# taintpro98/rnd-semantic-segmentation

Hardware: AMD Instinct MI355X
Metric: train images/sec at 769x769 bf16 (DeepLabV2-ResNet101 + ASPP) (higher is better)
Workload: dtype bf16; 1 GPU; train_src.py DeepLabV2-R101 bf16, 769x769 synthetic Cityscapes crops, batch 8 per GPU, 1xMI355X; global_batch=8, parallelism=dp1, weights=formula (synthetic), hip_graph_replay=False

## Files before the change

### rnd_semantic_segmentation_amd/csrc/elementwise.hip

```cpp
#include "mi_common.h"
#include <mutex>
#include <stdlib.h>
#include <string.h>

static thread_local char g_err[512] = "";

int mi_set_error(int code, const char* fmt, ...) {
    va_list ap;
    va_start(ap, fmt);
    vsnprintf(g_err, sizeof(g_err), fmt, ap);
    va_end(ap);
    return code;
}

const MiSwitches& mi_sw() {
    static MiSwitches sw;
    static std::once_flag once;
    std::call_once(once, [] {
        auto env = [](const char* name, int dflt) {
            const char* e = getenv(name);
            return e ? atoi(e) : dflt;
        };
        sw.igemm_staged = env("MI_IGEMM_STAGED", 1);
        sw.igemm_pp = env("MI_IGEMM_PP", 1);
        sw.igemm_pp_mink = env("MI_IGEMM_PP_MINK", 512);
        sw.igemm_mt = env("MI_IGEMM_MT", 0);
        sw.igemm_bn = env("MI_IGEMM_BN", 0);
        sw.igemm_pref = env("MI_IGEMM_PREF", 1);
        sw.pp_korder = env("MI_IGEMM_PP_KORDER", 1);
#ifdef MI_EXPERIMENTS
        sw.pp_loop = env("MI_IGEMM_PP_LOOP", 0);
#else
        sw.pp_loop = 0;
#endif
        sw.igemm_pw = env("MI_IGEMM_PW", 0);
        sw.wgrad_q3_slots = env("MI_WGRAD_Q3_SLOTS", 512);
        sw.wgrad_q3_slots_beside = env("MI_WGRAD_Q3_SLOTS_BESIDE", 448);
        sw.wgrad_s4_slots = env("MI_WGRAD_S4_SLOTS", 512);
        if (sw.wgrad_s4_slots < 64) sw.wgrad_s4_slots = 512;
        sw.wgrad_ti256 = env("MI_WGRAD_TI256", -1);
        sw.wgrad_p3 = env("MI_WGRAD_P3", 0);
        sw.wgrad_q3 = env("MI_WGRAD_Q3", 1);
        sw.wgrad_s4 = env("MI_WGRAD_S4", 1);
        sw.gconv_bn128 = env("MI_GCONV_BN128", 0);
        sw.gconv_kc = env("MI_GCONV_KC", 0);
        sw.gconv_remap = env("MI_GCONV_REMAP", 1);
        sw.gconv_ks2_wgs = env("MI_GCONV_KS2_WGS", 320);
        sw.gconv_kc32_wgs = env("MI_GCONV_KC32_WGS", 1536);
        sw.gconv_bn32_wgs = env("MI_GCONV_BN32_WGS", 256);
        sw.gconv_bn_any = env("MI_GCONV_BN_ANY", 1);
        sw.gconv_bn_c = env("MI_GCONV_BN_C", 64);
        sw.gconv_bn_force = env("MI_GCONV_BN_FORCE", 0);
        sw.gconv3_wgs = env("MI_GCONV3_WGS", 512);
#ifdef MI_EXPERIMENTS
        sw.gconv_dbg = env("MI_GC_DBG", 0);
        sw.gw_dbg = env("MI_GW_DBG", 0);
#else
        sw.gconv_dbg = sw.gw_dbg = 0;
#endif
        sw.gwm_steps = env("MI_GWM_STEPS", 48);
        if (sw.gwm_steps < 1) sw.gwm_steps = 48;
        sw.gwm_fused3 = env("MI_GWM_FUSED3", 1);
        sw.gwgrad3 = env("MI_GWGRAD3", 1);
#ifdef MI_EXPERIMENTS
        sw.p3_dbg = env("MI_P3_DBG", 0);
#else
        sw.p3_dbg = 0;
#endif
        sw.pp_trace_wg = env("MI_PP_TRACE_WG", 0);
        sw.stem_direct = env("MI_STEM_DIRECT", 1);
        sw.stem_pool_wgrad = env("MI_STEM_POOL_WGRAD", 1);
        sw.head_mask = env("MI_HEAD_MASK", 1);
        sw.sgd_pack = env("MI_SGD_PACK", 1);
        sw.stem_wgrad_splits = env("MI_STEM_WGRAD_SPLITS", 512);
        if (sw.stem_wgrad_splits < 1 || sw.stem_wgrad_splits > 4096) sw.stem_wgrad_splits = 512;
    });
// ... 337 lines not shown
```

### rnd_semantic_segmentation_amd/csrc/igemm_tn.hip

```cpp
#include "wgrad_common.h"
#include <stdlib.h>

namespace {

constexpr int TO = 128, TI = 128, KP = 64;
constexpr int ROWB = 256;
constexpr int TILE_BYTES = KP * ROWB;
constexpr int STAGE_BYTES = 2 * TILE_BYTES;
constexpr int LDS_BYTES = 2 * STAGE_BYTES;

__device__ __attribute__((aligned(256))) uint32_t g_zero_page_tn[64];

struct WgradParams {
    const __bf16* dY;
    const __bf16* X;
    float* slab;
    int M, O, I, T;
    int Ho, Wo, Ha, Wa;
    int ksz, stride, pad, dil;
    int S, rows_per_split;
    int o_tiles, i_tiles;
};

template <int OFF>
// ... 140 lines not shown
    const int wi = wave & 1, wo_ = wave >> 1;
    f32x4 acc[4][4];
#pragma unroll
    for (int a = 0; a < 4; ++a)
#pragma unroll
        for (int b = 0; b < 4; ++b) acc[a][b] = f32x4{0.f, 0.f, 0.f, 0.f};

    const int g = lane >> 4, q = (lane & 15) >> 2, pc = lane & 3;
    const int rsw = (((g & 1) * 4 + q) << 1);
    const int row_off = (g * 4 + q) * ROWB + (pc & 1) * 8;
    const unsigned lds0 = lds_address(smem);
    auto compute = [&](int buf) {
        const unsigned sy = lds0 + buf * STAGE_BYTES + row_off;
        const unsigned sx = sy + TILE_BYTES;
#pragma unroll
        for (int ks = 0; ks < 2; ++ks) tn_frag_mfma(sy + (ks * 32) * ROWB, sx + (ks * 32) * ROWB, wi, wo_, pc, rsw, acc);
    };

    if (nk > 0) {
        stage(0);
        asm volatile("s_waitcnt vmcnt(0)" ::: "memory");
        __syncthreads();
        for (int kt = 0; kt < nk; ++kt) {
            const int cur = kt & 1;
            if (kt + 1 < nk) stage(cur ^ 1);
            compute(cur);
            asm volatile("s_waitcnt vmcnt(0)" ::: "memory");
            __syncthreads();
        }
    }
    slab_store(p.slab + ((long)(split * p.T + t) * p.O) * p.I, p.I, p.O, p.I, o0 + wo_ * 64, i0 + wi * 64, lane, acc);
}

constexpr int KP4 = 32, SLOT4 = 2 * KP4 * ROWB, NSLOT4 = 4, LDS4_BYTES = NSLOT4 * SLOT4;

__global__ __launch_bounds__(256, 2) void wgrad_s4_kernel(WgradParams p) {
    extern __shared__ __attribute__((aligned(16))) char smem[];
    const int tid = threadIdx.x, lane = tid & 63;
    const int wave = __builtin_amdgcn_readfirstlane(tid >> 6);
    const WgDecode wg = wg_decode<TO, TI, KP4>(blockIdx.x, p.o_tiles * p.i_tiles * p.S, p.o_tiles, p.i_tiles, 1, p.M, p.rows_per_split);
    const int split = wg.split, o0 = wg.o0, i0 = wg.i0, m_begin = wg.m_begin, m_end = wg.m_end, nk = wg.nk;

    const int prow = lane >> 4, pch = lane & 15;
    const long rows = m_end > m_begin ? m_end - m_begin : 0;
    const __amdgpu_buffer_rsrc_t rs_y = __builtin_amdgcn_make_buffer_rsrc(const_cast<__bf16*>(p.dY + (long)m_begin * p.O), 0, (int)(rows * p.O * 2), 0x00020000);
    const __amdgpu_buffer_rsrc_t rs_x = __builtin_amdgcn_make_buffer_rsrc(const_cast<__bf16*>(p.X + (long)m_begin * p.I), 0, (int)(rows * p.I * 2), 0x00020000);
    unsigned vy[2], vx[2];
#pragma unroll
    for (int j = 0; j < 2; ++j) {
        const int row = (wave * 2 + j) * 4 + prow;
        const int lch = pch ^ ((row & 7) << 1);
        const int oc = o0 + lch * 8, ic = i0 + lch * 8;
        vy[j] = (unsigned)(((long)row * p.O + oc) * 2) | (oc < p.O ? 0u : 0x80000000u);
        vx[j] = (unsigned)(((long)row * p.I + ic) * 2) | (ic < p.I ? 0u : 0x80000000u);
    }
    const unsigned y_step = (unsigned)KP4 * p.O * 2, x_step = (unsigned)KP4 * p.I * 2;
    auto stage = [&](int slot) {
        char* sy = smem + slot * SLOT4 + wave * 2048;
        char* sx = sy + KP4 * ROWB;
#pragma unroll
        for (int j = 0; j < 2; ++j) {
            blds16_tn(rs_y, vy[j], sy + j * 1024);
            blds16_tn(rs_x, vx[j], sx + j * 1024);
            vy[j] += y_step;
            vx[j] += x_step;
        }
    };

    const int wi = wave & 1, wo_ = wave >> 1;
    f32x4 acc[4][4];
#pragma unroll
    for (int a = 0; a < 4; ++a)
#pragma unroll
        for (int b = 0; b < 4; ++b) acc[a][b] = f32x4{0.f, 0.f, 0.f, 0.f};
    const int g = lane >> 4, q = (lane & 15) >> 2, pc = lane & 3;
    const int rsw = (((g & 1) * 4 + q) << 1);
    const int row_off = (g * 4 + q) * ROWB + (pc & 1) * 8;
    const unsigned lds0 = lds_address(smem);
    auto compute = [&](int slot) {
        const unsigned sy = lds0 + slot * SLOT4 + row_off;
        tn_frag_mfma(sy, sy + KP4 * ROWB, wi, wo_, pc, rsw, acc);
    };

    stage(0);
    stage(1);
    stage(2);
    for (int s = 0; s < nk; ++s) {
        asm volatile("s_waitcnt vmcnt(8)" ::: "memory");
        __builtin_amdgcn_s_barrier();
        stage((s + 3) & (NSLOT4 - 1));
        compute(s & (NSLOT4 - 1));
    }
    slab_store(p.slab + ((long)split * p.O) * p.I, p.I, p.O, p.I, o0 + wo_ * 64, i0 + wi * 64, lane, acc);
}

constexpr int TI2 = 256, KP2 = 32;
constexpr int XROWB = 512;
constexpr int Y2_BYTES = KP2 * ROWB, X2_BYTES = KP2 * XROWB;
constexpr int STAGE2_BYTES = Y2_BYTES + X2_BYTES, NSTAGE2 = 3, LDS2_BYTES = NSTAGE2 * STAGE2_BYTES;

template <int MODE>
__global__ __launch_bounds__(256, 2) void wgrad_tn256_kernel(WgradParams p) {
    extern __shared__ __attribute__((aligned(16))) char smem[];
    const int tid = threadIdx.x, lane = tid & 63;
    const int wave = __builtin_amdgcn_readfirstlane(tid >> 6);
    const WgDecode wg = wg_decode<TO, TI2, KP2>(blockIdx.x, p.o_tiles * p.i_tiles * p.T * p.S, p.o_tiles, p.i_tiles, p.T, p.M, p.rows_per_split);
    const int t = wg.mid, split = wg.split, o0 = wg.o0, i0 = wg.i0, m_begin = wg.m_begin, m_end = wg.m_end, nk = wg.nk;
    const int ky = t / p.ksz, kx = t - ky * p.ksz;
    const char* zero = reinterpret_cast<const char*>(g_zero_page_tn);

    const int yrow_l = lane >> 4, ych = lane & 15, xrow_l = lane >> 5, xch = lane & 31;
    const int dys = ky * p.dil - p.pad, dxs = kx * p.dil - p.pad;
    int y_m[2], x_m[4], x_ho[4], x_wo[4];
    const char* y_ptr[2];
    const char* x_ptr[4];
    bool y_col[2], x_col[4];
    const int HoWo = p.Ho * p.Wo;
#pragma unroll
    for (int j = 0; j < 2; ++j) {
        const int row = (wave * 2 + j) * 4 + yrow_l;
        const int lch = ych ^ ((row & 7) << 1);
        y_m[j] = m_begin + row;
        y_col[j] = o0 + lch * 8 < p.O;
        y_ptr[j] = reinterpret_cast<const char*>(p.dY + (long)y_m[j] * p.O + o0 + lch * 8);
// ... 173 lines not shown
    wgrad_reduce_body(q.slab, q.dw, q.scale, q.S, q.T, q.O, q.I, q.accumulate, q.out_map, q.ncls, bx, o, tile);
}

constexpr int P3_KS = 64, P3_XROWS = 80;
constexpr int P3_DY_BYTES = P3_KS * ROWB, P3_X_BYTES = P3_XROWS * ROWB, P3_SLAB = P3_DY_BYTES + P3_X_BYTES;
constexpr int P3_LDS = 4 * P3_SLAB;
constexpr int P3_NPY = 4, P3_NPX = 5;

struct WgradP3Params {
    const __bf16* dY;
    const __bf16* X;
    float* slab;
    int O, I, H, W, d, WP, BH;
    long Q;
    int S, slabs_per_split;
    int o_tiles, i_tiles;
    int dbg;
};

#ifdef MI_EXPERIMENTS
#include "../../tools/experiments/wgrad_p3.inc"
#endif

constexpr int Q3_TO = 64;
constexpr int Q3_YROWB = 128;
constexpr int Q3_DY_BYTES = P3_KS * Q3_YROWB, Q3_STAGE = Q3_DY_BYTES + P3_X_BYTES;
constexpr int Q3_LDS = 2 * Q3_STAGE;

#ifdef MI_EXPERIMENTS
#define Q3_DBG(b) (p.dbg & (b))
#else
#define Q3_DBG(b) 0
#endif
__global__ __launch_bounds__(256, 2) void wgrad_q3_kernel(WgradP3Params p) {
    extern __shared__ __attribute__((aligned(16))) char smem[];
    const int tid = threadIdx.x, lane = tid & 63;
    const int wq = __builtin_amdgcn_readfirstlane(tid >> 6);
    const WgDecode wg = wg_decode_tile<Q3_TO, TI>(blockIdx.x, p.o_tiles * p.i_tiles * 3 * p.S, p.o_tiles, p.i_tiles, 3);
    const int ky = wg.mid, split = wg.split, o0 = wg.o0, i0 = wg.i0;
    const long q_begin = (long)split * p.slabs_per_split * P3_KS;
    long left = (p.Q - q_begin + P3_KS - 1) / P3_KS;
    const int ns = (int)(left < 0 ? 0 : (left < p.slabs_per_split ? left : p.slabs_per_split));
    const int Qi = (int)p.Q;
    const int n0 = P3_KS / p.WP, r0 = P3_KS - n0 * p.WP;
    const int pix_step = n0 * p.W + r0;

    const int yprow = lane >> 3, ypch = lane & 7;
    const char* yzero = reinterpret_cast<const char*>(g_zero_page_tn) + ypch * 16;
    const int yspan0 = wq * 16;
    const int ylch = ypch ^ ((((yspan0 + yprow) >> 1) & 3) << 1);
    const bool yok = o0 + ylch * 8 < p.O;
    const unsigned yrow_bytes = (unsigned)p.O * 2u;
    const unsigned yoff = yprow * yrow_bytes + (o0 + ylch * 8) * 2;
    const char* dy_b = reinterpret_cast<const char*>(p.dY);
    int y_q = (int)(q_begin + yspan0), y_wp, y_pix;
    {
        const int bh = y_q / p.WP;
        y_wp = y_q - bh * p.WP;
        y_pix = bh * p.W + y_wp - p.d;
    }
    const int xprow = lane >> 4, xpch = lane & 15;
    const char* xzero = reinterpret_cast<const char*>(g_zero_page_tn) + xpch * 16;
    const int dh = (ky - 1) * p.d;
    const int xspan0 = wq * 20;
    const int xlch_e = xpch ^ (((xspan0 + xprow) & 7) << 1), xlch_o = xpch ^ (((xspan0 + xprow + 4) & 7) << 1);
    const bool xok_e = i0 + xlch_e * 8 < p.I, xok_o = i0 + xlch_o * 8 < p.I;
    const unsigned xrow_bytes = (unsigned)p.I * 2u;
    const unsigned xoff_e = xprow * xrow_bytes + (i0 + xlch_e * 8) * 2, xoff_o = xprow * xrow_bytes + (i0 + xlch_o * 8) * 2;
    const char* x_b = reinterpret_cast<const char*>(p.X);
    int x_q = (int)(q_begin + xspan0 - p.d), x_wp, x_h, x_pix;
    {
        const long qs = (long)x_q + p.WP;
        const int bh = (int)(qs / p.WP) - 1;
        x_wp = (int)(qs % p.WP);
// ... 126 lines not shown
            } else {
#pragma unroll
                for (int b = 0; b < 4; ++b) asm volatile("" ::"v"(yf[b].v));
#pragma unroll
                for (int kx = 0; kx < 3; ++kx)
#pragma unroll
                    for (int a = 0; a < 2; ++a) asm volatile("" ::"v"(xf[kx][a].v));
            }
        }
    };

    if (ns > 0) {
        stage(0);
        asm volatile("s_waitcnt vmcnt(0)" ::: "memory");
        __syncthreads();
        for (int s = 0; s < ns; ++s) {
            const int cur = s & 1;
            if (s + 1 < ns && !Q3_DBG(1)) stage(cur ^ 1);
            compute(cur);
            asm volatile("s_waitcnt vmcnt(0)" ::: "memory");
            __syncthreads();
        }
    }

    if (Q3_DBG(8)) {
#pragma unroll
        for (int kx = 0; kx < 3; ++kx)
#pragma unroll
            for (int a = 0; a < 2; ++a)
#pragma unroll
                for (int b = 0; b < 4; ++b) asm volatile("" ::"v"(acc[kx][a][b]));
        return;
    }
#pragma unroll
    for (int kx = 0; kx < 3; ++kx) slab_store(p.slab + ((long)(split * 9 + ky * 3 + kx) * p.O) * p.I, p.I, p.O, p.I, o0, i0 + wq * 32, lane, acc[kx]);
}

struct P3Plan { int S, slabs_per_split; long Q; int WP, o_tiles, i_tiles; };
bool p3_plan(int B, int H, int W, int O, int I, int dil, bool force, P3Plan& pl, bool q3 = false, bool beside = false) {
    if (dil < 1 || dil > 8) return false;
    pl.WP = W + 2 * dil;
    pl.Q = (long)B * H * pl.WP;
    pl.o_tiles = q3 ? (O + Q3_TO - 1) / Q3_TO : (O + TO - 1) / TO;
    pl.i_tiles = (I + TI - 1) / TI;
    const long ns = (pl.Q + P3_KS - 1) / P3_KS;
    const int groups = pl.o_tiles * pl.i_tiles * 3;
    long S = (q3 ? (beside ? mi_sw().wgrad_q3_slots_beside : mi_sw().wgrad_q3_slots) : 256) / groups;
    if (S < 1) S = 1;
    if (S > ns) S = ns;
    pl.slabs_per_split = (int)((ns + S - 1) / S);
    pl.S = (int)((ns + pl.slabs_per_split - 1) / pl.slabs_per_split);
    if (P3_KS / pl.WP + 1 > H || pl.WP < 20 || pl.Q >= (1L << 31) - 4096) return false;
    if (force) return true;
    if (q3) return (long)O * I >= 256L * 256 && pl.slabs_per_split >= 8;
    return O >= 96 && I >= 96 && pl.slabs_per_split >= 8;
}

int pick_splits(long M, int tiles) { return wgrad_pick_splits(M, tiles, KP, 8, 6, 512, 64); }

}

extern "C" size_t mi_conv_wgrad_workspace(int B, int Ho, int Wo, int O, int I, int ksize) {
    const long M = (long)B * Ho * Wo;
    const int T = ksize * ksize;
    const int tiles = ((O + TO - 1) / TO) * ((I + TI - 1) / TI) * T;
    const int S = pick_splits(M, tiles);
    size_t need = (size_t)S * T * O * I * sizeof(float);
    if (I >= 256) {
        const int S2 = pick_splits256(M, ((O + TO - 1) / TO) * ((I + TI2 - 1) / TI2) * T);
        const size_t n2 = (size_t)S2 * T * O * I * sizeof(float);
        if (n2 > need) need = n2;
    }
    if (ksize == 1) {
        const size_t n4 = (size_t)(pick_splits256(M, tiles) > pick_splits_s4(M, tiles) ? pick_splits256(M, tiles) : pick_splits_s4(M, tiles)) * O * I * sizeof(float);
        if (n4 > need) need = n4;
    }
    if (ksize == 3) {
        P3Plan pl;
        for (int d = 1; d <= 8; d *= 2)
            for (int q3 = 0; q3 < 2; ++q3)
                if (p3_plan(B, Ho, Wo, O, I, d, true, pl, q3 != 0)) {
                    const size_t n3 = (size_t)pl.S * 9 * O * I * sizeof(float);
                    if (n3 > need) need = n3;
                }
    }
    return need;
}

template <auto KERN, int LDS, class P>
static void launch_lds(unsigned grid, unsigned block, hipStream_t st, const P& p) {
    static std::atomic<uint64_t> attr{0};
    mi_allow_dynamic_lds((const void*)KERN, LDS, attr);
    hipLaunchKernelGGL(KERN, dim3(grid), dim3(block), LDS, st, p);
}

static int launch_p3(const void* dy, const void* x, float* ws, int H, int W, int O, int I, int dil, const P3Plan& pl, int BH, hipStream_t st, bool q3 = false) {
    WgradP3Params q;
    q.dY = (const __bf16*)dy;
    q.X = (const __bf16*)x;
    q.slab = ws;
    q.O = O;
    q.I = I;
    q.H = H;
    q.W = W;
    q.d = dil;
    q.WP = pl.WP;
    q.BH = BH;
    q.Q = pl.Q;
    q.S = pl.S;
    q.slabs_per_split = pl.slabs_per_split;
    q.o_tiles = pl.o_tiles;
    q.i_tiles = pl.i_tiles;
    q.dbg = mi_sw().p3_dbg;
    const unsigned nb = (unsigned)(pl.o_tiles * pl.i_tiles * 3 * pl.S);
    if (q3) {
        launch_lds<wgrad_q3_kernel, Q3_LDS>(nb, 256, st, q);
        return 0;
    }
#ifdef MI_EXPERIMENTS
    launch_lds<wgrad_p3_kernel, P3_LDS>(nb, 512, st, q);
    return 0;
#else
    return -1;
#endif
}

struct WgradPlan {
    int kernel;
    int mode;
    int S;
    int steps;
    int step_rows;
    int o_tiles, i_tiles;
    int deferred;
    P3Plan p3;
};
static void wgrad_plan(int B, int Ha, int Wa, int I, int Ho, int Wo, int O, int ksize, int stride, int pad, int dil, int out_map, bool deferred,
                       size_t workspace_bytes, WgradPlan& w) {
    w = WgradPlan{};
    w.deferred = deferred;
    const long M = (long)B * Ho * Wo;
    const int T = ksize * ksize;
    const bool same = stride == 1 && Ha == Ho && Wa == Wo;
#ifdef MI_EXPERIMENTS
    const int p3_mode = mi_sw().wgrad_p3;
#else
    const int p3_mode = 0;
#endif
    const int q3_mode = mi_sw().wgrad_q3;
    const bool fused_ok = out_map == 0 && ksize == 3 && same && pad == dil;
    for (int q3 = 1; q3 >= 0; --q3) {
        const int mode = q3 ? (p3_mode ? 0 : q3_mode) : p3_mode;
        if (!fused_ok || !mode) continue;
        P3Plan pl;
        if (p3_plan(B, Ho, Wo, O, I, dil, mode == 2, pl, q3 != 0, q3 && deferred) && (size_t)pl.S * 9 * O * I * sizeof(float) <= workspace_bytes) {
            w.kernel = q3 ? MI_WPLAN_Q3 : MI_WPLAN_P3;
            w.S = pl.S;
            w.steps = pl.slabs_per_split;
            w.step_rows = P3_KS;
            w.o_tiles = pl.o_tiles;
            w.i_tiles = pl.i_tiles;
            w.p3 = pl;
            return;
        }
    }
    w.o_tiles = (O + TO - 1) / TO;
    const bool small32 = (long)M * (O > I ? O : I) * 2 < (1L << 31);
    const bool pointwise = same && ksize == 1 && pad == 0;
    if (use_tn256(O, I, ksize, pad, stride, Ha, Ho, Wa, Wo)) {
        w.kernel = MI_WPLAN_TN256;
        w.mode = pointwise ? 2 : 1;
        w.i_tiles = (I + TI2 - 1) / TI2;
        w.S = pick_splits256(M, w.o_tiles * w.i_tiles * T);
        w.step_rows = KP2;
    } else if (mi_sw().wgrad_s4 && pointwise && small32) {
        w.kernel = MI_WPLAN_S4;
        w.i_tiles = (I + TI - 1) / TI;
        w.S = pick_splits_s4(M, w.o_tiles * w.i_tiles);
        w.step_rows = KP4;
    } else {
        w.kernel = MI_WPLAN_TN;
        w.mode = pointwise && small32 ? 2 : (same ? 1 : 0);
        w.i_tiles = (I + TI - 1) / TI;
        w.S = pick_splits(M, w.o_tiles * w.i_tiles * T);
        w.step_rows = KP;
    }
    const long steps = (M + w.step_rows - 1) / w.step_rows;
    w.steps = (int)((steps + w.S - 1) / w.S);
}

extern "C" int mi_conv_wgrad_route(int B, int Ha, int Wa, int I, int Ho, int Wo, int O, int ksize, int stride, int pad, int dil, int out_map) {
    WgradPlan w;
    wgrad_plan(B, Ha, Wa, I, Ho, Wo, O, ksize, stride, pad, dil, out_map, false, mi_conv_wgrad_workspace(B, Ho, Wo, O, I, ksize), w);
    return w.kernel;
}

extern "C" int mi_conv_wgrad_plan(int B, int Ha, int Wa, int I, int Ho, int Wo, int O, int ksize, int stride, int pad, int dil, int out_map, int deferred,
                                  int* plan) {
    MI_REQUIRE(plan, "mi_conv_wgrad_plan: null plan");
    MI_REQUIRE(B > 0 && Ha > 0 && Wa > 0 && Ho > 0 && Wo > 0 && O > 0 && I > 0, "mi_conv_wgrad_plan: non-positive dimension");
    MI_REQUIRE(ksize == 1 || ksize == 3, "mi_conv_wgrad_plan: ksize");
    MI_REQUIRE(stride >= 1 && dil >= 1 && pad >= 0, "mi_conv_wgrad_plan: bad stride/dil/pad");
    WgradPlan w;
    wgrad_plan(B, Ha, Wa, I, Ho, Wo, O, ksize, stride, pad, dil, out_map, deferred != 0, mi_conv_wgrad_workspace(B, Ho, Wo, O, I, ksize), w);
    const int v[MI_WPLAN_LEN] = {w.kernel, w.mode, w.S, w.steps, w.step_rows, w.o_tiles, w.i_tiles, w.deferred};
    for (int k = 0; k < MI_WPLAN_LEN; ++k) plan[k] = v[k];
    return MI_OK;
}

static int wgrad_finish(WgradReduceJob* defer, hipStream_t stream, const float* slab, float* dw, const float* scale, int S, int T, int O, int I, int accumulate,
                        int out_map, int ncls, int o_real) {
    const int gx = (I + (T == 1 ? 255 : 63)) / (T == 1 ? 256 : 64);
    if (defer) {
        *defer = WgradReduceJob{slab, dw, scale, S, T, O, I, accumulate, out_map, ncls, gx, o_real};
        return MI_OK;
    }
    hipLaunchKernelGGL(wgrad_reduce_kernel, dim3((unsigned)gx, (unsigned)o_real), dim3(256), 0, stream, slab, dw, scale, S, T, O, I, accumulate, out_map, ncls);
    MI_CHECK_LAUNCH("mi_conv_wgrad reduce");
    return MI_OK;
}

static int mi_conv_wgrad_impl(const void* dy, const void* x, float* dw, int B, int Ha, int Wa, int I, int Ho, int Wo, int O,
                              int ksize, int stride, int pad, int dil, const float* scale_o, int accumulate, int out_map, int ncls,
                              size_t dw_elems, void* workspace, size_t workspace_bytes, void* stream, WgradReduceJob* defer) {
    MI_REQUIRE(dy && x && dw && workspace, "mi_conv_wgrad: null operand");
    MI_REQUIRE(B > 0 && Ha > 0 && Wa > 0 && Ho > 0 && Wo > 0, "mi_conv_wgrad: non-positive dimension");
    MI_REQUIRE(O % 8 == 0 && I % 8 == 0, "mi_conv_wgrad: O=%d, I=%d must be multiples of 8", O, I);
    MI_REQUIRE(ksize == 1 || ksize == 3, "mi_conv_wgrad: ksize");
    MI_REQUIRE(out_map == 0 || (out_map == 1 && ksize == 1), "mi_conv_wgrad: out_map 1 needs ksize 1");
    if (out_map == 1) {
        MI_REQUIRE(ncls > 0 && 36 * ncls <= MI_ASPP_KPAD && O >= 36 * ncls, "mi_conv_wgrad: out_map 1 needs 0 < 36*ncls=%d <= min(O=%d, %d)", 36 * ncls, O, MI_ASPP_KPAD);
        MI_REQUIRE(dw_elems >= (size_t)36 * ncls * I, "mi_conv_wgrad: dw holds %zu floats, the ASPP gradient needs %zu", dw_elems, (size_t)36 * ncls * I);
    } else {
        MI_REQUIRE(dw_elems >= (size_t)O * I * ksize * ksize, "mi_conv_wgrad: dw holds %zu floats, the gradient needs %zu", dw_elems, (size_t)O * I * ksize * ksize);
    }
    MI_REQUIRE(mi_aligned16(dy) && mi_aligned16(x) && mi_aligned16(workspace), "mi_conv_wgrad: alignment");
    const long M = (long)B * Ho * Wo;
    MI_REQUIRE(M < (1L << 31) && (long)B * Ha * Wa < (1L << 31), "mi_conv_wgrad: pixel count overflows int32");
    const size_t need = mi_conv_wgrad_workspace(B, Ho, Wo, O, I, ksize);
    if (workspace_bytes < need) return mi_set_error(MI_ENOMEM, "mi_conv_wgrad: workspace %zu < %zu", workspace_bytes, need);
    WgradPlan w;
    wgrad_plan(B, Ha, Wa, I, Ho, Wo, O, ksize, stride, pad, dil, out_map, defer != nullptr, workspace_bytes, w);
    if (w.kernel == MI_WPLAN_Q3 || w.kernel == MI_WPLAN_P3) {
        if (launch_p3(dy, x, (float*)workspace, Ho, Wo, O, I, dil, w.p3, B * Ho, (hipStream_t)stream, w.kernel == MI_WPLAN_Q3) != 0)
            return mi_set_error(MI_EINVAL, "mi_conv_wgrad: the 8-wave fused-row kernel exists in experiment builds only");
        MI_CHECK_LAUNCH("mi_conv_wgrad (fused 3x3 rows)");
        return wgrad_finish(defer, (hipStream_t)stream, (const float*)workspace, dw, scale_o, w.S, 9, O, I, accumulate, 0, 1, O);
    }
    WgradParams p;
    p.dY = (const __bf16*)dy;
    p.X = (const __bf16*)x;
    p.slab = (float*)workspace;
    p.M = (int)M;
    p.O = O;
    p.I = I;
    p.T = ksize * ksize;
    p.Ho = Ho;
    p.Wo = Wo;
    p.Ha = Ha;
    p.Wa = Wa;
    p.ksz = ksize;
    p.stride = stride;
    p.pad = pad;
    p.dil = dil;
    p.o_tiles = w.o_tiles;
    p.i_tiles = w.i_tiles;
    p.S = w.S;
    p.rows_per_split = w.steps * w.step_rows;
    const hipStream_t sq = (hipStream_t)stream;
    const unsigned nb = (unsigned)(p.o_tiles * p.i_tiles * p.T * p.S);
    if (w.kernel == MI_WPLAN_TN256) {
        if (w.mode == 2) launch_lds<wgrad_tn256_kernel<2>, LDS2_BYTES>(nb, 256, sq, p);
        else launch_lds<wgrad_tn256_kernel<1>, LDS2_BYTES>(nb, 256, sq, p);
        MI_CHECK_LAUNCH("mi_conv_wgrad (128 x 256 tile)");
    } else if (w.kernel == MI_WPLAN_S4) {
        launch_lds<wgrad_s4_kernel, LDS4_BYTES>(nb, 256, sq, p);
        MI_CHECK_LAUNCH("mi_conv_wgrad (1x1 deep stream)");
    } else {
        if (w.mode == 2) launch_lds<wgrad_tn_kernel<2>, LDS_BYTES>(nb, 256, sq, p);
        else if (w.mode == 1) launch_lds<wgrad_tn_kernel<1>, LDS_BYTES>(nb, 256, sq, p);
        else launch_lds<wgrad_tn_kernel<0>, LDS_BYTES>(nb, 256, sq, p);
        MI_CHECK_LAUNCH("mi_conv_wgrad");
    }
    int o_real = O;
    if (out_map == 1) o_real = 36 * ncls;
    else ncls = 1;
    return wgrad_finish(defer, (hipStream_t)stream, p.slab, dw, scale_o, p.S, p.T, O, I, accumulate, out_map, ncls, o_real);
}

extern "C" int mi_conv_wgrad(const void* dy, const void* x, float* dw, int B, int Ha, int Wa, int I, int Ho, int Wo, int O,
                             int ksize, int stride, int pad, int dil, const float* scale_o, int accumulate, int out_map, int ncls,
                             size_t dw_elems, void* workspace, size_t workspace_bytes, void* stream) {
    return mi_conv_wgrad_impl(dy, x, dw, B, Ha, Wa, I, Ho, Wo, O, ksize, stride, pad, dil, scale_o, accumulate, out_map, ncls, dw_elems, workspace, workspace_bytes,
                              stream, nullptr);
}

extern "C" size_t mi_conv_wgrad_job_bytes(void) { return sizeof(WgradReduceJob); }
extern "C" int mi_conv_wgrad_partial(const void* dy, const void* x, float* dw, int B, int Ha, int Wa, int I, int Ho, int Wo, int O,
                                     int ksize, int stride, int pad, int dil, const float* scale_o, int accumulate, int out_map, int ncls,
                                     size_t dw_elems, void* workspace, size_t workspace_bytes, void* job, void* stream) {
    MI_REQUIRE(job, "mi_conv_wgrad_partial: null job");
    return mi_conv_wgrad_impl(dy, x, dw, B, Ha, Wa, I, Ho, Wo, O, ksize, stride, pad, dil, scale_o, accumulate, out_map, ncls, dw_elems, workspace, workspace_bytes,
                              stream, (WgradReduceJob*)job);
}
extern "C" int mi_conv_wgrad_reduce(const void* jobs, int n, void* stream) {
    MI_REQUIRE(jobs && n >= 1 && n <= MI_REDUCE_MAX_JOBS, "mi_conv_wgrad_reduce: 1 .. %d jobs", MI_REDUCE_MAX_JOBS);
    WgradReduceTable tab;
    tab.n = n;
    int total = 0;
// ... 13 lines not shown
```

### rnd_semantic_segmentation_amd/csrc/mi_common.h

```cpp
#pragma once
#include <hip/hip_runtime.h>
#include <stdint.h>
#include <stdio.h>
#include <stdarg.h>
#include <atomic>
#include "../../include/mi355seg.h"

typedef __attribute__((ext_vector_type(8))) __bf16 bf16x8;
typedef __attribute__((ext_vector_type(4))) __bf16 bf16x4;
typedef __attribute__((ext_vector_type(2))) __bf16 bf16x2;
typedef __attribute__((ext_vector_type(4))) float f32x4;
typedef __attribute__((ext_vector_type(4))) short s16x4;
typedef __attribute__((ext_vector_type(4))) uint32_t u32x4;
typedef __attribute__((ext_vector_type(2))) uint32_t u32x2;

int mi_set_error(int code, const char* fmt, ...);

struct MiSwitches {
    int igemm_staged;
    int igemm_pp;
    int igemm_pp_mink;
    int igemm_mt;
    int igemm_bn;
    int igemm_pref;
    int pp_korder;
    int pp_loop;
    int igemm_pw;
    int wgrad_q3_slots;
    int wgrad_q3_slots_beside;
    int wgrad_s4_slots;
    int wgrad_ti256;
    int wgrad_p3;
    int wgrad_q3;
    int wgrad_s4;
    int gconv_bn128;
    int gconv_kc;
    int gconv_remap;
    int gconv_ks2_wgs;
    int gconv_kc32_wgs;
    int gconv_bn32_wgs;
    int gconv_bn_any;
    int gconv_bn_c;
    int gconv_bn_force;
    int gconv3_wgs;
    int gconv_dbg;
    int gw_dbg;
    int gwm_steps;
    int gwm_fused3;
    int gwgrad3;
    int p3_dbg;
    int pp_trace_wg;
    int stem_wgrad_splits;
    int stem_direct;
    int stem_pool_wgrad;
    int sgd_pack;
    int head_mask;
};
const MiSwitches& mi_sw();

struct MiConvStats {
    float* partial;
    const float* pilot;
    int nparts;
};
int mi_conv_gemm_impl(const void* a, const void* wp, void* out, int B, int Ha, int Wa, int Ca, int Ho, int Wo, int N, int ksize, int stride, int pad,
                      int dil, int gather_mode, const float* scale, const float* bias, const void* res, const void* msk, void* mask_out, int flags,
                      int zgw, float alpha, void* stream, MiConvStats* st);
// ... 115 lines not shown
```

Baseline: 307.8 images/s.

## Pair K-ranges inside 512-thread wgrad workgroups with LDS reduction

Adds a KG=2 variant of the 1x1 (S4) and Q3 weight-gradient kernels in which two 4-wave groups in one 512-thread workgroup process adjacent K (row) ranges and sum their accumulators through LDS before a single slab store. The number of split partials written to global memory and later reduced is halved. Controlled by MI_WGRAD_KGROUPS bits; by default only the S4 path is paired. The cost is doubled LDS per workgroup, lower occupancy bounds, and an extra LDS reduction step.

```diff
diff --git a/rnd_semantic_segmentation_amd/csrc/elementwise.hip b/rnd_semantic_segmentation_amd/csrc/elementwise.hip
--- a/rnd_semantic_segmentation_amd/csrc/elementwise.hip
+++ b/rnd_semantic_segmentation_amd/csrc/elementwise.hip
@@ -42,6 +42,7 @@
         sw.wgrad_p3 = env("MI_WGRAD_P3", 0);
         sw.wgrad_q3 = env("MI_WGRAD_Q3", 1);
         sw.wgrad_s4 = env("MI_WGRAD_S4", 1);
+        sw.wgrad_kgroups = env("MI_WGRAD_KGROUPS", 1);
         sw.gconv_bn128 = env("MI_GCONV_BN128", 0);
         sw.gconv_kc = env("MI_GCONV_KC", 0);
         sw.gconv_remap = env("MI_GCONV_REMAP", 1);
diff --git a/rnd_semantic_segmentation_amd/csrc/igemm_tn.hip b/rnd_semantic_segmentation_amd/csrc/igemm_tn.hip
--- a/rnd_semantic_segmentation_amd/csrc/igemm_tn.hip
+++ b/rnd_semantic_segmentation_amd/csrc/igemm_tn.hip
@@ -196,13 +196,45 @@
     slab_store(p.slab + ((long)(split * p.T + t) * p.O) * p.I, p.I, p.O, p.I, o0 + wo_ * 64, i0 + wi * 64, lane, acc);
 }
 
+template <int KP_>
+__device__ __forceinline__ void kgroup_range(WgDecode& w, int grp, int M, int rows_per_split) {
+    const long m0 = (long)(2 * w.split) * rows_per_split, mb = m0 + (long)grp * rows_per_split;
+    const long r0 = M - m0 < rows_per_split ? M - m0 : rows_per_split;
+    w.nk = r0 > 0 ? (int)((r0 + KP_ - 1) / KP_) : 0;
+    w.m_begin = (int)(mb < M ? mb : M);
+    w.m_end = (int)(mb + rows_per_split < M ? mb + rows_per_split : M);
+}
+__device__ __forceinline__ f32x4* kgroup_slot(char* rings, int w4, int n, int lane) {
+    asm volatile("s_waitcnt vmcnt(0)" ::: "memory");
+    __syncthreads();
+    return reinterpret_cast<f32x4*>(rings) + (w4 * n) * 64 + lane;
+}
+template <int NA, int NB>
+__device__ __forceinline__ void kgroup_put(f32x4* mine, const f32x4 (&acc)[NA][NB]) {
+#pragma unroll
+    for (int a = 0; a < NA; ++a)
+#pragma unroll
+        for (int b = 0; b < NB; ++b) mine[(a * NB + b) * 64] = acc[a][b];
+}
+template <int NA, int NB>
+__device__ __forceinline__ void kgroup_add(const f32x4* mine, f32x4 (&acc)[NA][NB]) {
+#pragma unroll
+    for (int a = 0; a < NA; ++a)
+#pragma unroll
+        for (int b = 0; b < NB; ++b) acc[a][b] = acc[a][b] + mine[(a * NB + b) * 64];
+}
+
 constexpr int KP4 = 32, SLOT4 = 2 * KP4 * ROWB, NSLOT4 = 4, LDS4_BYTES = NSLOT4 * SLOT4;
 
-__global__ __launch_bounds__(256, 2) void wgrad_s4_kernel(WgradParams p) {
-    extern __shared__ __attribute__((aligned(16))) char smem[];
+template <int KG>
+__global__ __launch_bounds__(256 * KG, 3 - KG) void wgrad_s4_kernel(WgradParams p) {
+    extern __shared__ __attribute__((aligned(16))) char smem_all[];
     const int tid = threadIdx.x, lane = tid & 63;
-    const int wave = __builtin_amdgcn_readfirstlane(tid >> 6);
-    const WgDecode wg = wg_decode<TO, TI, KP4>(blockIdx.x, p.o_tiles * p.i_tiles * p.S, p.o_tiles, p.i_tiles, 1, p.M, p.rows_per_split);
+    const int wave8 = __builtin_amdgcn_readfirstlane(tid >> 6);
+    const int grp = KG == 2 ? wave8 >> 2 : 0, wave = wave8 & 3;
+    char* smem = smem_all + grp * LDS4_BYTES;
+    WgDecode wg = wg_decode<TO, TI, KP4>(blockIdx.x, p.o_tiles * p.i_tiles * p.S, p.o_tiles, p.i_tiles, 1, p.M, p.rows_per_split);
+    if (KG == 2) kgroup_range<KP4>(wg, grp, p.M, p.rows_per_split);
     const int split = wg.split, o0 = wg.o0, i0 = wg.i0, m_begin = wg.m_begin, m_end = wg.m_end, nk = wg.nk;
 
     const int prow = lane >> 4, pch = lane & 15;
@@ -254,6 +286,13 @@
         __builtin_amdgcn_s_barrier();
         stage((s + 3) & (NSLOT4 - 1));
         compute(s & (NSLOT4 - 1));
+    }
+    if (KG == 2) {
+        f32x4* mine = kgroup_slot(smem_all, wave, 16, lane);
+        if (grp) kgroup_put(mine, acc);
+        __syncthreads();
+        if (grp) return;
+        kgroup_add(mine, acc);
     }
     slab_store(p.slab + ((long)split * p.O) * p.I, p.I, p.O, p.I, o0 + wo_ * 64, i0 + wi * 64, lane, acc);
 }
@@ -493,14 +532,18 @@
 #else
 #define Q3_DBG(b) 0
 #endif
-__global__ __launch_bounds__(256, 2) void wgrad_q3_kernel(WgradP3Params p) {
-    extern __shared__ __attribute__((aligned(16))) char smem[];
+template <int KG>
+__global__ __launch_bounds__(256 * KG, 3 - KG) void wgrad_q3_kernel(WgradP3Params p) {
+    extern __shared__ __attribute__((aligned(16))) char smem_all[];
     const int tid = threadIdx.x, lane = tid & 63;
-    const int wq = __builtin_amdgcn_readfirstlane(tid >> 6);
+    const int wave8 = __builtin_amdgcn_readfirstlane(tid >> 6);
+    const int grp = KG == 2 ? wave8 >> 2 : 0, wq = wave8 & 3;
+    char* smem = smem_all + grp * Q3_LDS;
     const WgDecode wg = wg_decode_tile<Q3_TO, TI>(blockIdx.x, p.o_tiles * p.i_tiles * 3 * p.S, p.o_tiles, p.i_tiles, 3);
     const int ky = wg.mid, split = wg.split, o0 = wg.o0, i0 = wg.i0;
-    const long q_begin = (long)split * p.slabs_per_split * P3_KS;
-    long left = (p.Q - q_begin + P3_KS - 1) / P3_KS;
+    const long q_first = (long)(KG * split) * p.slabs_per_split * P3_KS;
+    const long q_begin = q_first + (long)grp * p.slabs_per_split * P3_KS;
+    long left = (p.Q - q_first + P3_KS - 1) / P3_KS;
     const int ns = (int)(left < 0 ? 0 : (left < p.slabs_per_split ? left : p.slabs_per_split));
     const int Qi = (int)p.Q;
     const int n0 = P3_KS / p.WP, r0 = P3_KS - n0 * p.WP;
@@ -693,11 +736,21 @@
                 for (int b = 0; b < 4; ++b) asm volatile("" ::"v"(acc[kx][a][b]));
         return;
     }
+    if (KG == 2) {
+        f32x4* mine = kgroup_slot(smem_all, wq, 24, lane);
+#pragma unroll
+        for (int kx = 0; kx < 3; ++kx)
+            if (grp) kgroup_put(mine + kx * 8 * 64, acc[kx]);
+        __syncthreads();
+        if (grp) return;
+#pragma unroll
+        for (int kx = 0; kx < 3; ++kx) kgroup_add(mine + kx * 8 * 64, acc[kx]);
+    }
 #pragma unroll
     for (int kx = 0; kx < 3; ++kx) slab_store(p.slab + ((long)(split * 9 + ky * 3 + kx) * p.O) * p.I, p.I, p.O, p.I, o0, i0 + wq * 32, lane, acc[kx]);
 }
 
-struct P3Plan { int S, slabs_per_split; long Q; int WP, o_tiles, i_tiles; };
+struct P3Plan { int S, slabs_per_split; long Q; int WP, o_tiles, i_tiles; bool kgroups; };
 bool p3_plan(int B, int H, int W, int O, int I, int dil, bool force, P3Plan& pl, bool q3 = false, bool beside = false) {
     if (dil < 1 || dil > 8) return false;
     pl.WP = W + 2 * dil;
@@ -709,9 +762,12 @@
     long S = (q3 ? (beside ? mi_sw().wgrad_q3_slots_beside : mi_sw().wgrad_q3_slots) : 256) / groups;
     if (S < 1) S = 1;
     if (S > ns) S = ns;
+    pl.kgroups = q3 && (mi_sw().wgrad_kgroups & 2) != 0;
+    if (pl.kgroups && S > 1) S &= ~1L;
     pl.slabs_per_split = (int)((ns + S - 1) / S);
     pl.S = (int)((ns + pl.slabs_per_split - 1) / pl.slabs_per_split);
-    if (P3_KS / pl.WP + 1 > H || pl.WP < 20 || pl.Q >= (1L << 31) - 4096) return false;
+    if (pl.kgroups) pl.S = (pl.S + 1) / 2;
+    if (P3_KS / pl.WP + 1 > H || pl.WP < 20 || pl.Q + (pl.kgroups ? (long)pl.slabs_per_split * P3_KS : 0) >= (1L << 31) - 4096) return false;
     if (force) return true;
     if (q3) return (long)O * I >= 256L * 256 && pl.slabs_per_split >= 8;
     return O >= 96 && I >= 96 && pl.slabs_per_split >= 8;
@@ -775,7 +831,8 @@
     q.dbg = mi_sw().p3_dbg;
     const unsigned nb = (unsigned)(pl.o_tiles * pl.i_tiles * 3 * pl.S);
     if (q3) {
-        launch_lds<wgrad_q3_kernel, Q3_LDS>(nb, 256, st, q);
+        if (pl.kgroups) launch_lds<wgrad_q3_kernel<2>, 2 * Q3_LDS>(nb, 512, st, q);
+        else launch_lds<wgrad_q3_kernel<1>, Q3_LDS>(nb, 256, st, q);
         return 0;
     }
 #ifdef MI_EXPERIMENTS
@@ -794,8 +851,16 @@
     int step_rows;
     int o_tiles, i_tiles;
     int deferred;
+    int kgroups;
     P3Plan p3;
 };
+static void wgrad_pair_ranges(long M, WgradPlan& w) {
+    const long steps = (M + w.step_rows - 1) / w.step_rows;
+    const int ranges = w.S > 1 ? w.S & ~1 : 1;
+    w.steps = (int)((steps + ranges - 1) / ranges);
+    w.S = (int)(((steps + w.steps - 1) / w.steps + 1) / 2);
+    w.kgroups = 1;
+}
 static void wgrad_plan(int B, int Ha, int Wa, int I, int Ho, int Wo, int O, int ksize, int stride, int pad, int dil, int out_map, bool deferred,
                        size_t workspace_bytes, WgradPlan& w) {
     w = WgradPlan{};
@@ -822,6 +887,7 @@
             w.o_tiles = pl.o_tiles;
             w.i_tiles = pl.i_tiles;
             w.p3 = pl;
+            w.kgroups = pl.kgroups;
             return;
         }
     }
@@ -848,6 +914,7 @@
     }
     const long steps = (M + w.step_rows - 1) / w.step_rows;
     w.steps = (int)((steps + w.S - 1) / w.S);
+    if (w.kernel == MI_WPLAN_S4 && (mi_sw().wgrad_kgroups & 1)) wgrad_pair_ranges(M, w);
 }
 
 extern "C" int mi_conv_wgrad_route(int B, int Ha, int Wa, int I, int Ho, int Wo, int O, int ksize, int stride, int pad, int dil, int out_map) {
@@ -935,7 +1002,8 @@
         else launch_lds<wgrad_tn256_kernel<1>, LDS2_BYTES>(nb, 256, sq, p);
         MI_CHECK_LAUNCH("mi_conv_wgrad (128 x 256 tile)");
     } else if (w.kernel == MI_WPLAN_S4) {
-        launch_lds<wgrad_s4_kernel, LDS4_BYTES>(nb, 256, sq, p);
+        if (w.kgroups) launch_lds<wgrad_s4_kernel<2>, 2 * LDS4_BYTES>(nb, 512, sq, p);
+        else launch_lds<wgrad_s4_kernel<1>, LDS4_BYTES>(nb, 256, sq, p);
         MI_CHECK_LAUNCH("mi_conv_wgrad (1x1 deep stream)");
     } else {
         if (w.mode == 2) launch_lds<wgrad_tn_kernel<2>, LDS_BYTES>(nb, 256, sq, p);
diff --git a/rnd_semantic_segmentation_amd/csrc/mi_common.h b/rnd_semantic_segmentation_amd/csrc/mi_common.h
--- a/rnd_semantic_segmentation_amd/csrc/mi_common.h
+++ b/rnd_semantic_segmentation_amd/csrc/mi_common.h
@@ -33,6 +33,7 @@
     int wgrad_p3;
     int wgrad_q3;
     int wgrad_s4;
+    int wgrad_kgroups;
     int gconv_bn128;
     int gconv_kc;
     int gconv_remap;
```

Result: no change. 307.3 images/s (-0.2%).

## Add fused-row 3x3 weight-gradient kernel for small channel counts

Applied to the files above, without the earlier changes.

Adds a new wgrad kernel for 3x3 stride-1 convolutions where both input and output channels fit in one tile (at most Q3_TO). Each block computes all three kx taps for one ky row over a range of flattened padded rows. It stages dY and a shifted X window into LDS through a 4-slot async pipeline and feeds 16x16x32 bf16 MFMAs. The planner tries it before the generic paths, and workspace sizing grows to hold its split slabs. It targets the small-channel 3x3 layers (e.g. 64-channel ResNet stages), where the tiled kernels waste most of a 128-wide tile.

```diff
diff --git a/rnd_semantic_segmentation_amd/csrc/elementwise.hip b/rnd_semantic_segmentation_amd/csrc/elementwise.hip
--- a/rnd_semantic_segmentation_amd/csrc/elementwise.hip
+++ b/rnd_semantic_segmentation_amd/csrc/elementwise.hip
@@ -42,6 +42,9 @@
         sw.wgrad_p3 = env("MI_WGRAD_P3", 0);
         sw.wgrad_q3 = env("MI_WGRAD_Q3", 1);
         sw.wgrad_s4 = env("MI_WGRAD_S4", 1);
+        sw.wgrad_taps64 = env("MI_WGRAD_TAPS64", 1);
+        sw.wgrad_taps64_slots = env("MI_WGRAD_TAPS64_SLOTS", 512);
+        if (sw.wgrad_taps64_slots < 3) sw.wgrad_taps64_slots = 512;
         sw.gconv_bn128 = env("MI_GCONV_BN128", 0);
         sw.gconv_kc = env("MI_GCONV_KC", 0);
         sw.gconv_remap = env("MI_GCONV_REMAP", 1);
diff --git a/rnd_semantic_segmentation_amd/csrc/igemm_tn.hip b/rnd_semantic_segmentation_amd/csrc/igemm_tn.hip
--- a/rnd_semantic_segmentation_amd/csrc/igemm_tn.hip
+++ b/rnd_semantic_segmentation_amd/csrc/igemm_tn.hip
@@ -697,7 +697,180 @@
     for (int kx = 0; kx < 3; ++kx) slab_store(p.slab + ((long)(split * 9 + ky * 3 + kx) * p.O) * p.I, p.I, p.O, p.I, o0, i0 + wq * 32, lane, acc[kx]);
 }
 
+constexpr int T64_XROWS = 80;
+constexpr int T64_DY_BYTES = P3_KS * Q3_YROWB, T64_X_BYTES = T64_XROWS * Q3_YROWB, T64_STAGE = T64_DY_BYTES + T64_X_BYTES;
+constexpr int T64_NSLOT = 4, T64_LDS = T64_NSLOT * T64_STAGE;
+constexpr int T64_MAX_S = 256;
+
+__global__ __launch_bounds__(256, 2) void wgrad_t64_kernel(WgradP3Params p) {
+    extern __shared__ __attribute__((aligned(16))) char smem[];
+    const int tid = threadIdx.x, lane = tid & 63;
+    const int wq = __builtin_amdgcn_readfirstlane(tid >> 6);
+    const WgDecode wg = wg_decode_tile<Q3_TO, TI>(blockIdx.x, 3 * p.S, 1, 1, 3);
+    const int ky = wg.mid, split = wg.split;
+    const long q_begin = (long)split * p.slabs_per_split * P3_KS;
+    const long left = (p.Q - q_begin + P3_KS - 1) / P3_KS;
+    const int ns = (int)(left < 0 ? 0 : (left < p.slabs_per_split ? left : p.slabs_per_split));
+    const int n0 = P3_KS / p.WP, r0 = P3_KS - n0 * p.WP;
+    const int dh = (ky - 1) * p.d;
+    const int nxp = (P3_KS + 2 * p.d + 7) >> 3;
+
+    const int prow = lane >> 3, pch = lane & 7;
+    const int lch = pch ^ (((prow >> 1) & 3) << 1);
+    const bool yok = lch * 8 < p.O, xok = lch * 8 < p.I;
+    const unsigned yrow_bytes = (unsigned)p.O * 2u, xrow_bytes = (unsigned)p.I * 2u;
+    const char* zero = reinterpret_cast<const char*>(g_zero_page_tn);
+    const char* dy_b = reinterpret_cast<const char*>(p.dY) + lch * 16;
+    const char* x_b = reinterpret_cast<const char*>(p.X) + lch * 16;
+    struct Row { int wp, bh, h; };
+    auto row_at = [&](long q) {
+        const unsigned qs = (unsigned)(q + p.WP), bh1 = qs / (unsigned)p.WP;
+        Row r;
+        r.bh = (int)bh1 - 1;
+        r.wp = (int)(qs - bh1 * (unsigned)p.WP);
+        r.h = r.bh < 0 ? p.H - 1 : (int)((unsigned)r.bh % (unsigned)p.H);
+        return r;
+    };
+    auto advance = [&](Row& r) {
+        r.wp += r0;
+        const int c = r.wp >= p.WP ? 1 : 0;
+        r.wp -= c ? p.WP : 0;
+        r.bh += n0 + c;
+        r.h += n0 + c;
+        r.h -= r.h >= p.H ? p.H : 0;
+    };
+    Row yr[2], xr[3];
+#pragma unroll
+    for (int j = 0; j < 2; ++j) yr[j] = row_at(q_begin + (wq * 2 + j) * 8 + prow);
+#pragma unroll
+    for (int j = 0; j < 3; ++j) xr[j] = row_at(q_begin + (wq + 4 * j) * 8 + prow - p.d);
+
+    auto stage = [&](int slot) {
+        char* ydst = smem + slot * T64_STAGE + wq * 2048;
+        char* xdst = smem + slot * T64_STAGE + T64_DY_BYTES + wq * 1024;
+#pragma unroll
+        for (int j = 0; j < 2; ++j) {
+            Row& r = yr[j];
+            const bool ok = yok && (unsigned)(r.wp - p.d) < (unsigned)p.W && (unsigned)r.bh < (unsigned)p.BH;
+            const int pix = r.bh * p.W + r.wp - p.d;
+            glds16_tn(ok ? dy_b + (unsigned long)(unsigned)pix * yrow_bytes : zero, ydst + j * 1024);
+            advance(r);
+        }
+#pragma unroll
+        for (int j = 0; j < 3; ++j) {
+            if (wq + 4 * j >= nxp) continue;
+            Row& r = xr[j];
+            const bool ok = xok && (unsigned)(r.wp - p.d) < (unsigned)p.W && (unsigned)r.bh < (unsigned)p.BH && (unsigned)(r.h + dh) < (unsigned)p.H;
+            const int pix = (r.bh + dh) * p.W + r.wp - p.d;
+            glds16_tn(ok ? x_b + (unsigned long)(unsigned)pix * xrow_bytes : zero, xdst + j * 4096);
+            advance(r);
+        }
+    };
+
+    f32x4 acc[3][1][4];
+#pragma unroll
+    for (int kx = 0; kx < 3; ++kx)
+#pragma unroll
+        for (int b = 0; b < 4; ++b) acc[kx][0][b] = f32x4{0.f, 0.f, 0.f, 0.f};
+    const int g = lane >> 4, q4 = (lane & 15) >> 2, pc = lane & 3;
+    const int rk0 = g * 4 + q4;
+    const unsigned y_off = rk0 * Q3_YROWB + (pc >> 1) * 16 + (pc & 1) * 8;
+    const int y_sw = (rk0 >> 1) & 3;
+    unsigned x_off[3];
+#pragma unroll
+    for (int kx = 0; kx < 3; ++kx) {
+        const int rk = rk0 + kx * p.d;
+        x_off[kx] = T64_DY_BYTES + rk * Q3_YROWB + ((wq ^ ((rk >> 1) & 3)) << 5) + (pc >> 1) * 16 + (pc & 1) * 8;
+    }
+    const unsigned lds0 = lds_address(smem);
+    auto compute = [&](int slot) {
+        unsigned sb = lds0 + slot * T64_STAGE;
+        asm volatile("" : "+v"(sb));
+#pragma unroll
+        for (int ks = 0; ks < 2; ++ks) {
+            union { bf16x8 v; s16x4 h[2]; } yf[4], xf[3];
+            if (Q3_DBG(2)) {
+#pragma unroll
+                for (int b = 0; b < 4; ++b) yf[b].h[0] = yf[b].h[1] = s16x4{(short)lane, 1, 2, 3};
+#pragma unroll
+                for (int kx = 0; kx < 3; ++kx) xf[kx].h[0] = xf[kx].h[1] = s16x4{(short)lane, 3, 2, 1};
+            }
+            if (!Q3_DBG(2)) {
+#pragma unroll
+            for (int b = 0; b < 4; ++b) {
+                const unsigned base = sb + y_off + ((b ^ y_sw) << 5);
+                if (ks == 0) {
+                    yf[b].h[0] = tr_read_lds<0>(base);
+                    yf[b].h[1] = tr_read_lds<16 * Q3_YROWB>(base);
+                } else {
+                    yf[b].h[0] = tr_read_lds<32 * Q3_YROWB>(base);
+                    yf[b].h[1] = tr_read_lds<48 * Q3_YROWB>(base);
+                }
+            }
+#pragma unroll
+            for (int kx = 0; kx < 3; ++kx) {
+                const unsigned base = sb + x_off[kx];
+                if (ks == 0) {
+                    xf[kx].h[0] = tr_read_lds<0>(base);
+                    xf[kx].h[1] = tr_read_lds<16 * Q3_YROWB>(base);
+                } else {
+                    xf[kx].h[0] = tr_read_lds<32 * Q3_YROWB>(base);
+                    xf[kx].h[1] = tr_read_lds<48 * Q3_YROWB>(base);
+                }
+            }
+            }
+            asm volatile("s_waitcnt lgkmcnt(0)" ::: "memory");
+            __builtin_amdgcn_sched_barrier(0);
+            if (!Q3_DBG(4)) {
+#pragma unroll
+            for (int kx = 0; kx < 3; ++kx)
+#pragma unroll
+                for (int b = 0; b < 4; ++b) acc[kx][0][b] = __builtin_amdgcn_mfma_f32_16x16x32_bf16(xf[kx].v, yf[b].v, acc[kx][0][b], 0, 0, 0);
+            } else {
+#pragma unroll
+                for (int b = 0; b < 4; ++b) asm volatile("" ::"v"(yf[b].v));
+#pragma unroll
+                for (int kx = 0; kx < 3; ++kx) asm volatile("" ::"v"(xf[kx].v));
+            }
+        }
+    };
+
+    stage(0);
+    if (ns > 1) stage(1);
+    if (ns > 2) stage(2);
+    for (int s = 0; s < ns; ++s) {
+        const int younger = ns - 1 - s;
+        if (younger >= 2) asm volatile("s_waitcnt vmcnt(8)" ::: "memory");
+        else if (younger == 1) asm volatile("s_waitcnt vmcnt(4)" ::: "memory");
+        else asm volatile("s_waitcnt vmcnt(0)" ::: "memory");
+        __builtin_amdgcn_s_barrier();
+        if (s + 3 < ns && !Q3_DBG(1)) stage((s + 3) & (T64_NSLOT - 1));
+        compute(s & (T64_NSLOT - 1));
+    }
+    if (Q3_DBG(8)) {
+#pragma unroll
+        for (int kx = 0; kx < 3; ++kx)
+#pragma unroll
+            for (int b = 0; b < 4; ++b) asm volatile("" ::"v"(acc[kx][0][b]));
+        return;
+    }
+#pragma unroll
+    for (int kx = 0; kx < 3; ++kx) slab_store(p.slab + ((long)(split * 9 + ky * 3 + kx) * p.O) * p.I, p.I, p.O, p.I, 0, wq * 16, lane, acc[kx]);
+}
+
 struct P3Plan { int S, slabs_per_split; long Q; int WP, o_tiles, i_tiles; };
+bool t64_plan(int B, int H, int W, int O, int I, int dil, P3Plan& pl) {
+    if (!mi_sw().wgrad_taps64 || O > Q3_TO || I > Q3_TO || dil < 1 || 2 * dil > T64_XROWS - P3_KS) return false;
+    pl.WP = W + 2 * dil;
+    pl.Q = (long)B * H * pl.WP;
+    pl.o_tiles = pl.i_tiles = 1;
+    if (P3_KS / pl.WP + 1 > H || pl.Q >= (1L << 31) - 4096) return false;
+    const long ns = (pl.Q + P3_KS - 1) / P3_KS;
+    const int S = wgrad_pick_splits(pl.Q, 3, P3_KS, 8, 6, mi_sw().wgrad_taps64_slots, T64_MAX_S);
+    pl.slabs_per_split = (int)((ns + S - 1) / S);
+    pl.S = (int)((ns + pl.slabs_per_split - 1) / pl.slabs_per_split);
+    return true;
+}
 bool p3_plan(int B, int H, int W, int O, int I, int dil, bool force, P3Plan& pl, bool q3 = false, bool beside = false) {
     if (dil < 1 || dil > 8) return false;
     pl.WP = W + 2 * dil;
@@ -744,6 +917,11 @@
                     const size_t n3 = (size_t)pl.S * 9 * O * I * sizeof(float);
                     if (n3 > need) need = n3;
                 }
+        if (mi_sw().wgrad_taps64 && O <= Q3_TO && I <= Q3_TO) {
+            const long ns = ((long)B * Ho * (Wo + T64_XROWS - P3_KS) + P3_KS - 1) / P3_KS, smax = ns > 7 ? (ns - 1) / 7 : 1;
+            const size_t n6 = (size_t)(smax < T64_MAX_S ? smax : T64_MAX_S) * 9 * O * I * sizeof(float);
+            if (n6 > need) need = n6;
+        }
     }
     return need;
 }
@@ -755,7 +933,7 @@
     hipLaunchKernelGGL(KERN, dim3(grid), dim3(block), LDS, st, p);
 }
 
-static int launch_p3(const void* dy, const void* x, float* ws, int H, int W, int O, int I, int dil, const P3Plan& pl, int BH, hipStream_t st, bool q3 = false) {
+static int launch_p3(const void* dy, const void* x, float* ws, int H, int W, int O, int I, int dil, const P3Plan& pl, int BH, hipStream_t st, int kind) {
     WgradP3Params q;
     q.dY = (const __bf16*)dy;
     q.X = (const __bf16*)x;
@@ -774,8 +952,12 @@
     q.i_tiles = pl.i_tiles;
     q.dbg = mi_sw().p3_dbg;
     const unsigned nb = (unsigned)(pl.o_tiles * pl.i_tiles * 3 * pl.S);
-    if (q3) {
+    if (kind == 1) {
         launch_lds<wgrad_q3_kernel, Q3_LDS>(nb, 256, st, q);
+        return 0;
+    }
+    if (kind == 2) {
+        launch_lds<wgrad_t64_kernel, T64_LDS>(nb, 256, st, q);
         return 0;
     }
 #ifdef MI_EXPERIMENTS
@@ -794,6 +976,7 @@
     int step_rows;
     int o_tiles, i_tiles;
     int deferred;
+    int taps64;
     P3Plan p3;
 };
 static void wgrad_plan(int B, int Ha, int Wa, int I, int Ho, int Wo, int O, int ksize, int stride, int pad, int dil, int out_map, bool deferred,
@@ -825,6 +1008,21 @@
             return;
         }
     }
+    if (fused_ok) {
+        P3Plan pl;
+        if (t64_plan(B, Ho, Wo, O, I, dil, pl) && (size_t)pl.S * 9 * O * I * sizeof(float) <= workspace_bytes) {
+            w.kernel = MI_WPLAN_TN;
+            w.mode = 1;
+            w.taps64 = 1;
+            w.S = pl.S;
+            w.steps = pl.slabs_per_split;
+            w.step_rows = P3_KS;
+            w.o_tiles = pl.o_tiles;
+            w.i_tiles = pl.i_tiles;
+            w.p3 = pl;
+            return;
+        }
+    }
     w.o_tiles = (O + TO - 1) / TO;
     const bool small32 = (long)M * (O > I ? O : I) * 2 < (1L << 31);
     const bool pointwise = same && ksize == 1 && pad == 0;
@@ -902,8 +1100,8 @@
     if (workspace_bytes < need) return mi_set_error(MI_ENOMEM, "mi_conv_wgrad: workspace %zu < %zu", workspace_bytes, need);
     WgradPlan w;
     wgrad_plan(B, Ha, Wa, I, Ho, Wo, O, ksize, stride, pad, dil, out_map, defer != nullptr, workspace_bytes, w);
-    if (w.kernel == MI_WPLAN_Q3 || w.kernel == MI_WPLAN_P3) {
-        if (launch_p3(dy, x, (float*)workspace, Ho, Wo, O, I, dil, w.p3, B * Ho, (hipStream_t)stream, w.kernel == MI_WPLAN_Q3) != 0)
+    if (w.kernel == MI_WPLAN_Q3 || w.kernel == MI_WPLAN_P3 || w.taps64) {
+        if (launch_p3(dy, x, (float*)workspace, Ho, Wo, O, I, dil, w.p3, B * Ho, (hipStream_t)stream, w.taps64 ? 2 : (w.kernel == MI_WPLAN_Q3 ? 1 : 0)) != 0)
             return mi_set_error(MI_EINVAL, "mi_conv_wgrad: the 8-wave fused-row kernel exists in experiment builds only");
         MI_CHECK_LAUNCH("mi_conv_wgrad (fused 3x3 rows)");
         return wgrad_finish(defer, (hipStream_t)stream, (const float*)workspace, dw, scale_o, w.S, 9, O, I, accumulate, 0, 1, O);
diff --git a/rnd_semantic_segmentation_amd/csrc/mi_common.h b/rnd_semantic_segmentation_amd/csrc/mi_common.h
--- a/rnd_semantic_segmentation_amd/csrc/mi_common.h
+++ b/rnd_semantic_segmentation_amd/csrc/mi_common.h
@@ -33,6 +33,8 @@
     int wgrad_p3;
     int wgrad_q3;
     int wgrad_s4;
+    int wgrad_taps64;
+    int wgrad_taps64_slots;
     int gconv_bn128;
     int gconv_kc;
     int gconv_remap;
```

Result: slower. 302.5 images/s before, 299.5 images/s after (-1.0%).
